# TrackieWay-OSS/TrackieLLM

Measured on AMD Instinct MI355X. Metric: cortex cycles/sec (frame+1s audio+128 tok), higher is better.
Workload: dtype int8 x q4_K/q6_K (i32 acc, f32 scales); 1 GPU; configs[3] fused cycle: YOLOv8n 640x640 frame (preprocess+network+NMS) + 1 s PCM (VAD + Whisper-tiny.en log-mel/encoder/16 forced decoder steps) + Mistral-7B Q4_K_M 64-token prefill and 128-token greedy decode, 3 concurrent HIP streams; concurrent_cycles_per_gpu=768, decode_groups=3, rows_per_llm_pass=256, layers=32, parallelism=replicas x1

## Files before the change

### include/tk/tk_audio.h

```cpp
#ifndef TK_MI355X_AUDIO_H
#define TK_MI355X_AUDIO_H

#include "tk_types.h"

#ifdef __cplusplus
extern "C" {
#endif

typedef struct tk_asr_whisper_context_s tk_asr_whisper_context_t;

typedef struct {
    tk_path_t* model_path;
    const char* language;
    bool translate_to_en;
    uint32_t sample_rate;
    void* user_data;
    int n_threads;
    int max_context;
    float word_threshold;
} tk_asr_whisper_config_t;

typedef struct {
    char* text;
    size_t text_length;
// ... 35 lines not shown
TK_API TK_NODISCARD tk_error_code_t tk_vad_silero_create(tk_vad_silero_context_t** out_context, const tk_vad_silero_config_t* config);
TK_API void tk_vad_silero_destroy(tk_vad_silero_context_t** context);
TK_API TK_NODISCARD tk_error_code_t tk_vad_silero_process_audio(tk_vad_silero_context_t* context, const int16_t* audio_data, size_t frame_count,
                                                                float* out_probability);
TK_API TK_NODISCARD tk_error_code_t tk_vad_silero_process_audio_with_events(tk_vad_silero_context_t* context, const int16_t* audio_data,
                                                                            size_t frame_count, tk_vad_silero_event_callback_t callback,
                                                                            void* user_data);
TK_API TK_NODISCARD tk_error_code_t tk_vad_silero_get_state(tk_vad_silero_context_t* context, tk_vad_silero_state_t* out_state);
TK_API TK_NODISCARD tk_error_code_t tk_vad_silero_reset(tk_vad_silero_context_t* context);
TK_API TK_NODISCARD tk_error_code_t tk_vad_silero_set_threshold(tk_vad_silero_context_t* context, float threshold);

typedef struct {
    int32_t n_mels, n_audio_ctx, n_audio_state, n_audio_head, n_audio_layer;
    int32_t n_text_ctx, n_text_state, n_text_head, n_text_layer, n_vocab;
} tk_mi355x_whisper_hparams_t;
TK_API TK_NODISCARD tk_error_code_t tk_mi355x_asr_create(tk_asr_whisper_context_t** out, const tk_mi355x_whisper_hparams_t* hp, uint64_t seed,
                                                         int device, int max_batch);
TK_API TK_NODISCARD tk_error_code_t tk_mi355x_asr_transcribe_tokens(tk_asr_whisper_context_t* ctx, int batch, const int16_t* pcm, int n_samples,
                                                                    int n_steps, int32_t* tokens_out, float* mel_out, float* enc_out,
                                                                    float* logits_out);
TK_API void tk_mi355x_asr_set_decode_steps(tk_asr_whisper_context_t* ctx, int n_steps);
TK_API TK_NODISCARD tk_error_code_t tk_mi355x_asr_set_reference_decode(tk_asr_whisper_context_t* ctx, int enable);
TK_API TK_NODISCARD tk_error_code_t tk_mi355x_asr_set_fast_contraction(tk_asr_whisper_context_t* ctx, int on);
TK_API TK_NODISCARD tk_error_code_t tk_mi355x_asr_transcribe_ref(tk_asr_whisper_context_t* ctx, const int16_t* pcm, int n_samples, int n_steps, float temperature,
                                                                 uint64_t seed, int32_t* tokens_out, float* logprobs_out, int32_t* result_len, int32_t* status);
TK_API int32_t tk_mi355x_asr_suppress_table(tk_asr_whisper_context_t* ctx, uint8_t* out, int32_t cap, int32_t* token_beg, int32_t* token_eot);
TK_API void tk_mi355x_asr_share_stats(const tk_asr_whisper_context_t* ctx, uint64_t* handles, uint64_t* batches, uint64_t* utterances, uint64_t* widest);
TK_API TK_NODISCARD tk_error_code_t tk_mi355x_asr_transcribe_policy(tk_asr_whisper_context_t* ctx, int batch, const int16_t* pcm, int n_samples,
                                                                    int n_steps, float temperature, uint64_t seed, int32_t* tokens_out,
                                                                    float* logprobs_out);
TK_API TK_NODISCARD tk_error_code_t tk_mi355x_asr_set_decode_policy(tk_asr_whisper_context_t* ctx, int enable, float temperature_inc,
                                                                    float entropy_thold, float logprob_thold, uint64_t seed);
TK_API void tk_mi355x_asr_last_decode(const tk_asr_whisper_context_t* ctx, float* temperature, float* avg_logprob, int32_t* attempts);
TK_API int tk_mi355x_asr_prompt_tokens(tk_asr_whisper_context_t* ctx, int32_t* out, int cap);
TK_API TK_NODISCARD tk_error_code_t tk_mi355x_asr_get_hparams(tk_asr_whisper_context_t* ctx, tk_mi355x_whisper_hparams_t* out);
TK_API TK_NODISCARD tk_error_code_t tk_mi355x_whisper_ggml_probe(const char* path, tk_mi355x_whisper_hparams_t* out, int32_t* n_tokens,
                                                                 int32_t* n_tensors);
TK_API TK_NODISCARD tk_error_code_t tk_mi355x_vad_onnx_probe(const char* path, int32_t* n_nodes, int32_t* n_initialisers, int32_t* n_state_inputs);
TK_API int tk_mi355x_vad_step(tk_vad_silero_context_t* ctx, float probability);
TK_API TK_NODISCARD tk_error_code_t tk_mi355x_vad_probabilities(tk_vad_silero_context_t* ctx, const float* windows, int n, float* out);

#ifdef __cplusplus
}
#endif
#endif
```

### trackiellm_amd/audio.py

```python
import ctypes as C

import numpy as np

from ._lib import check, lib
from .llm import _Path


class WhisperHP(C.Structure):
    _fields_ = [(n, C.c_int32) for n in ("n_mels", "n_audio_ctx", "n_audio_state", "n_audio_head", "n_audio_layer",
                                         "n_text_ctx", "n_text_state", "n_text_head", "n_text_layer", "n_vocab")]


def WHISPER_TINY_EN():
    return WhisperHP(80, 1500, 384, 6, 4, 448, 384, 6, 4, 51864)


class _AsrConfig(C.Structure):
    _fields_ = [("model_path", C.POINTER(_Path)), ("language", C.c_char_p), ("translate_to_en", C.c_bool), ("sample_rate", C.c_uint32),
                ("user_data", C.c_void_p), ("n_threads", C.c_int), ("max_context", C.c_int), ("word_threshold", C.c_float)]


class AsrResult(C.Structure):
    _fields_ = [("text", C.c_char_p), ("text_length", C.c_size_t), ("confidence", C.c_float), ("is_partial", C.c_bool)]

# ... 39 lines not shown
    def transcribe_policy(self, pcm, n_steps, temperature=0.0, seed=0):
        pcm = np.ascontiguousarray(pcm, np.int16)
        B, n = pcm.shape
        toks = np.zeros((B, n_steps), np.int32)
        lp = np.zeros((B, n_steps), np.float32)
        check(lib().tk_mi355x_asr_transcribe_policy(self.h, B, pcm.ctypes.data_as(C.c_void_p), n, n_steps, C.c_float(temperature), C.c_uint64(seed),
                                                    toks.ctypes.data_as(C.c_void_p), lp.ctypes.data_as(C.c_void_p)))
        return toks, lp

    def set_decode_policy(self, enable=True, temperature_inc=0.2, entropy_thold=2.4, logprob_thold=-1.0, seed=0):
        check(lib().tk_mi355x_asr_set_decode_policy(self.h, int(enable), C.c_float(temperature_inc), C.c_float(entropy_thold),
                                                    C.c_float(logprob_thold), C.c_uint64(seed)))

    def last_decode(self):
        t, a, n = C.c_float(0), C.c_float(0), C.c_int32(0)
        lib().tk_mi355x_asr_last_decode(self.h, C.byref(t), C.byref(a), C.byref(n))
        return t.value, a.value, n.value

    def set_reference_decode(self, enable=True):
        check(lib().tk_mi355x_asr_set_reference_decode(self.h, int(enable)))

    def set_fast_contraction(self, on=True):
        check(lib().tk_mi355x_asr_set_fast_contraction(self.h, 1 if on else 0))

    def transcribe_ref(self, pcm, n_steps, temperature=0.0, seed=0):
        pcm = np.ascontiguousarray(pcm, np.int16).reshape(-1)
        toks = np.zeros(n_steps, np.int32)
        lp = np.zeros(n_steps, np.float32)
        rl, st = C.c_int32(0), C.c_int32(0)
        check(lib().tk_mi355x_asr_transcribe_ref(self.h, pcm.ctypes.data_as(C.c_void_p), pcm.size, n_steps, C.c_float(temperature), C.c_uint64(seed),
                                                 toks.ctypes.data_as(C.c_void_p), lp.ctypes.data_as(C.c_void_p), C.byref(rl), C.byref(st)))
        return toks, lp, rl.value, st.value

    def suppress_table(self):
        beg, eot = C.c_int32(0), C.c_int32(0)
        n = lib().tk_mi355x_asr_suppress_table(self.h, None, 0, C.byref(beg), C.byref(eot))
        if n <= 0:
            return None, 0, 0
        tab = np.zeros(n, np.uint8)
        lib().tk_mi355x_asr_suppress_table(self.h, tab.ctypes.data_as(C.c_void_p), n, C.byref(beg), C.byref(eot))
        return tab, beg.value, eot.value

    def share_stats(self):
        v = [C.c_uint64(0) for _ in range(4)]
        lib().tk_mi355x_asr_share_stats(self.h, *[C.byref(x) for x in v])
        return tuple(int(x.value) for x in v)
# ... 184 lines not shown
```

### trackiellm_amd/csrc/abi/tk_abi_audio.cpp

```cpp
#include <math.h>
#include <stdio.h>
#include <stdlib.h>
#include <string.h>
#include <unistd.h>

#include <memory>
#include <string>
#include <vector>

#include "../audio/tk_audio_engine.h"
#include "../audio/tk_vad_graph.h"
#include "../audio/tk_whisper_ggml.h"
#include "tk/tk_audio.h"
#include "tk/tk_mi355x_ext.h"

#define TK_ASR_MAX_BUFFER (16000 * 30)

static tk_error_code_t afail(tk_error_code_t code, const std::string& why) {
    tk_error_set_detail("%s", why.c_str());
    return code;
}

static uint64_t seed_of(const std::string& p, uint64_t dflt) {
    size_t k = p.find("seed=");
// ... 4 lines not shown
static std::string file_identity(const std::string& path) {
    struct stat st;
    if (path.compare(0, 12, "synthetic://") == 0 || stat(path.c_str(), &st) != 0) return path;
    return path + "|" + std::to_string((long long)st.st_size) + "|" + std::to_string((long long)st.st_mtim.tv_sec) + "." + std::to_string((long long)st.st_mtim.tv_nsec) + "|" +
           std::to_string((unsigned long long)st.st_ino);
}

#include <chrono>
#include <condition_variable>
#include <deque>
#include <map>
#include <mutex>
#include <thread>

#define TK_ASR_SHARED_MAX_BATCH 32

struct AsrReq {
    const int16_t* pcm = nullptr;
    int n_samples = 0, n_steps = 0;
    std::vector<int32_t> prompt;
    bool policy = false;
    bool ref = false;
    bool fast = false;
    float temperature = 0.0f;
    uint64_t seed = 0;
    int32_t* tokens = nullptr;
    float* logprobs = nullptr;
    int32_t result_len = 0, status = 0;
    bool ok = false, done = false;
    std::string err;
};

struct SharedAsr {
    std::string key;
    TkWhisperModel model;
    std::vector<std::string> vocab;
    std::vector<uint8_t> suppress;
    int32_t token_beg = 0, token_eot = 0;
    std::unique_ptr<TkAsr> eng;
    bool scheduled = false;
    std::mutex mu;
    std::condition_variable cv_req, cv_done;
    std::deque<AsrReq*> q;
    std::thread th;
    bool stop = false;
    int handles = 0;
// ... 15 lines not shown
        if (eng && eng->max_batch >= want) return true;
        std::unique_ptr<TkAsr> ne(new TkAsr());
        if (!ne->init(&model, want)) { *err = ne->error; return false; }
        eng.swap(ne);
        return true;
    }
    void run() {
        std::unique_lock<std::mutex> lk(mu);
        for (;;) {
            cv_req.wait(lk, [&] { return stop || !q.empty(); });
            if (stop) break;
            if (handles > 1 && !q.front()->policy) {
                const auto until = std::chrono::steady_clock::now() + std::chrono::microseconds(1000);
                while ((int)q.size() < (handles < TK_ASR_SHARED_MAX_BATCH ? handles : TK_ASR_SHARED_MAX_BATCH) && !stop)
                    if (cv_req.wait_until(lk, until) == std::cv_status::timeout) break;
                if (stop) break;
            }
            std::vector<AsrReq*> job;
            AsrReq* first = q.front();
            if (first->policy) { job.push_back(first); q.pop_front(); }
            else
                for (auto it = q.begin(); it != q.end() && (int)job.size() < TK_ASR_SHARED_MAX_BATCH;) {
                    AsrReq* r = *it;
                    if (!r->policy && r->ref == first->ref && r->fast == first->fast && r->n_steps == first->n_steps && r->prompt == first->prompt) { job.push_back(r); it = q.erase(it); }
                    else ++it;
                }
            int cap = 1;
            while (cap < (int)job.size() || (cap < handles && cap < TK_ASR_SHARED_MAX_BATCH)) cap *= 2;
            lk.unlock();
            std::string err;
            std::unique_lock<std::mutex> el(eng_mu);
            bool ok = ensure_engine(cap, &err);
            if (ok) {
                eng->fast = first->fast;
                const int B = (int)job.size();
                int n_max = 0;
                for (AsrReq* r : job) n_max = r->n_samples > n_max ? r->n_samples : n_max;
                if (first->ref) {
                    std::vector<int16_t> pcm((size_t)B * (n_max > 0 ? n_max : 1), 0);
                    std::vector<int32_t> lens(B), toks((size_t)B * first->n_steps), rl(B), stt(B);
                    std::vector<float> lps((size_t)B * first->n_steps);
                    for (int b = 0; b < B; ++b) {
                        lens[b] = job[b]->n_samples;
                        if (job[b]->n_samples > 0) memcpy(&pcm[(size_t)b * n_max], job[b]->pcm, (size_t)job[b]->n_samples * sizeof(int16_t));
                    }
                    ok = eng->transcribe_ref(B, pcm.data(), n_max, lens.data(), first->prompt.data(), (int)first->prompt.size(), first->n_steps, first->temperature, first->seed,
                                             suppress.data(), token_beg, token_eot, toks.data(), lps.data(), rl.data(), stt.data());
                    for (int b = 0; ok && b < B; ++b) {
                        memcpy(job[b]->tokens, &toks[(size_t)b * first->n_steps], (size_t)first->n_steps * sizeof(int32_t));
                        if (job[b]->logprobs) memcpy(job[b]->logprobs, &lps[(size_t)b * first->n_steps], (size_t)first->n_steps * sizeof(float));
                        job[b]->result_len = rl[b];
                        job[b]->status = stt[b];
                    }
                } else if (first->policy) {
                    ok = eng->transcribe_policy(1, first->pcm, first->n_samples, first->prompt.data(), (int)first->prompt.size(), first->n_steps, first->temperature, first->seed,
                                                first->tokens, first->logprobs);
                } else if (B == 1) {
// ... 23 lines not shown
    }
    void submit(AsrReq* r) {
        std::unique_lock<std::mutex> lk(mu);
        q.push_back(r);
        cv_req.notify_all();
        cv_done.wait(lk, [&] { return r->done; });
    }
};

static std::mutex g_asr_mu;
static std::map<std::string, std::weak_ptr<SharedAsr>> g_asr_registry;

struct tk_asr_whisper_context_s {
    std::shared_ptr<SharedAsr> sh;
    std::vector<int16_t> buffer;
    size_t buffer_size = 0;
    bool has_partial = false;
    std::string last_text, language;
    int decode_steps = 16;
    int32_t sot = 0, nots = 0, eot = 0;
    bool multilingual = false, translate = false;
    bool forced_greedy = false;
    bool fast = false;
    bool policy_on = false;
    float temperature_inc = 0.2f, entropy_thold = 2.4f, logprob_thold = -1.0f;
    uint64_t policy_seed = 0;
    float last_temperature = 0.0f, last_avg_logprob = 0.0f;
    int last_attempts = 0;
    ~tk_asr_whisper_context_s() {
        if (sh) { std::lock_guard<std::mutex> lk(sh->mu); sh->handles--; }
    }
};

static const char* const k_whisper_langs[] = {
    "en", "zh", "de", "es", "ru", "ko", "fr", "ja", "pt", "tr", "pl", "ca", "nl", "ar", "sv", "it", "id", "hi", "fi", "vi", "he", "uk", "el", "ms", "cs",
    "ro", "da", "hu", "ta", "no", "th", "ur", "hr", "bg", "lt", "la", "mi", "ml", "cy", "sk", "te", "fa", "lv", "bn", "sr", "az", "sl", "kn", "et", "mk",
    "br", "eu", "is", "hy", "ne", "mn", "bs", "kk", "sq", "sw", "gl", "mr", "pa", "si", "km", "sn", "yo", "so", "af", "oc", "ka", "be", "tg", "sd", "gu",
    "am", "yi", "lo", "uz", "fo", "ht", "ps", "tk", "nn", "mt", "sa", "lb", "my", "bo", "tl", "mg", "as", "tt", "haw", "ln", "ha", "ba", "jw", "su", "yue"};

static int whisper_lang_id(const std::string& code) {
    for (int i = 0; i < (int)(sizeof k_whisper_langs / sizeof k_whisper_langs[0]); ++i)
        if (code == k_whisper_langs[i]) return i;
    return -1;
}

static bool asr_prompt(const tk_asr_whisper_context_s* c, std::vector<int32_t>* out, std::string* why, bool timestamps = false) {
// ... 102 lines not shown
    c->sot = 50257 + ml < v - 3 ? 50257 + ml : v - 3;
    c->nots = 50362 + ml < v - 1 ? 50362 + ml : v - 1;
    c->eot = 50256 + ml < v - 4 ? 50256 + ml : v - 4;
    c->multilingual = ml != 0;
    if (ml) {
        const int n_lang = v - 51865 + 99;
        c->eot = 50257; c->sot = 50258;
        c->nots = c->sot + 1 + n_lang + 5;
    }
    { std::lock_guard<std::mutex> hl(sh->mu); build_suppress(sh.get(), c.get()); }
    *out = c.release();
    return TK_SUCCESS;
}

static tk_error_code_t asr_run_ref(tk_asr_whisper_context_s* c, const int16_t* pcm, int n_samples, const std::vector<int32_t>& prompt, int n_steps, float temperature,
                                   uint64_t seed, int32_t* tokens_out, float* logprobs_out, int32_t* result_len, int32_t* status) {
    SharedAsr* sh = c->sh.get();
    const TkWhisperHP& h = sh->model.hp;
    if (sh->suppress.empty()) return afail(TK_ERROR_INFERENCE_FAILED, "this vocabulary has no timestamp tokens: the reference-parameter decode does not apply");
    if (n_samples < 0 || n_samples > h.n_samples()) return afail(TK_ERROR_INFERENCE_FAILED, "audio longer than the model window");
    if (prompt.empty() || (int)prompt.size() + n_steps > h.n_text_ctx) return afail(TK_ERROR_INFERENCE_FAILED, "prompt + steps exceed the text context");
    if (sh->scheduled) {
        AsrReq r;
        r.pcm = pcm; r.n_samples = n_samples; r.n_steps = n_steps; r.prompt = prompt; r.ref = true; r.fast = c->fast; r.policy = temperature > 0.0f; r.temperature = temperature; r.seed = seed;
        r.tokens = tokens_out; r.logprobs = logprobs_out;
        sh->submit(&r);
        if (!r.ok) return afail(TK_ERROR_INFERENCE_FAILED, r.err);
        if (result_len) *result_len = r.result_len;
        if (status) *status = r.status;
        return TK_SUCCESS;
    }
    std::lock_guard<std::mutex> lk(sh->eng_mu);
    const int32_t len = n_samples;
    int32_t rl = 0, stt = 0;
    sh->eng->fast = c->fast;
    if (!sh->eng->transcribe_ref(1, pcm, n_samples, &len, prompt.data(), (int)prompt.size(), n_steps, temperature, seed, sh->suppress.data(), sh->token_beg, sh->token_eot,
                                 tokens_out, logprobs_out, &rl, &stt))
        return afail(TK_ERROR_INFERENCE_FAILED, sh->eng->error);
    if (result_len) *result_len = rl;
    if (status) *status = stt;
    return TK_SUCCESS;
}

static tk_error_code_t asr_run(tk_asr_whisper_context_s* c, int batch, const int16_t* pcm, int n_samples, const std::vector<int32_t>& prompt, int n_steps, bool policy,
                               float temperature, uint64_t seed, int32_t* tokens_out, float* logprobs_out, std::vector<float>* mel, std::vector<float>* enc,
                               std::vector<float>* lg) {
    SharedAsr* sh = c->sh.get();
    if (sh->scheduled && batch == 1 && !mel && !enc && !lg) {
        AsrReq r;
        r.pcm = pcm; r.n_samples = n_samples; r.n_steps = n_steps; r.prompt = prompt; r.fast = c->fast; r.policy = policy; r.temperature = temperature; r.seed = seed;
        r.tokens = tokens_out; r.logprobs = logprobs_out;
        const TkWhisperHP& h = sh->model.hp;
        if (n_samples < 0 || n_samples > h.n_samples()) return afail(TK_ERROR_INFERENCE_FAILED, "audio longer than the model window");
        if (prompt.empty() || (int)prompt.size() + n_steps > h.n_text_ctx) return afail(TK_ERROR_INFERENCE_FAILED, "prompt + steps exceed the text context");
        sh->submit(&r);
        return r.ok ? TK_SUCCESS : afail(TK_ERROR_INFERENCE_FAILED, r.err);
    }
    std::lock_guard<std::mutex> lk(sh->eng_mu);
    std::string err;
    if (!sh->ensure_engine(batch, &err)) return afail(TK_ERROR_GPU_MEMORY, err);
    sh->eng->fast = c->fast;
    const bool ok = policy ? sh->eng->transcribe_policy(batch, pcm, n_samples, prompt.data(), (int)prompt.size(), n_steps, temperature, seed, tokens_out, logprobs_out)
                           : sh->eng->transcribe(batch, pcm, n_samples, prompt.data(), (int)prompt.size(), n_steps, tokens_out, mel, enc, lg);
    return ok ? TK_SUCCESS : afail(TK_ERROR_INFERENCE_FAILED, sh->eng->error);
}

extern "C" {

tk_error_code_t tk_asr_whisper_create(tk_asr_whisper_context_t** out_context, const tk_asr_whisper_config_t* config) {
    if (!out_context || !config || !config->model_path || !config->model_path->path_str) return TK_ERROR_INVALID_ARGUMENT;
    if (config->sample_rate != 16000) return afail(TK_ERROR_INVALID_ARGUMENT, "Whisper needs 16 kHz audio");
    const std::string path = config->model_path->path_str;
    tk_error_code_t rc = asr_new(out_context, tk_whisper_tiny_en(), path, seed_of(path, 6), tk_mi355x_get_default_device(), 1, true);
    if (rc == TK_SUCCESS && config->language) (*out_context)->language = config->language;
    if (rc == TK_SUCCESS) (*out_context)->translate = config->translate_to_en;
    const char* pol = getenv("TK_MI355X_ASR_POLICY");
    if (rc == TK_SUCCESS && pol && pol[0] == '1') (*out_context)->policy_on = true;
    return rc;
}

tk_error_code_t tk_mi355x_asr_create(tk_asr_whisper_context_t** out, const tk_mi355x_whisper_hparams_t* hp, uint64_t seed, int device, int max_batch) {
    if (!out || !hp) return TK_ERROR_INVALID_ARGUMENT;
    TkWhisperHP h{hp->n_mels, hp->n_audio_ctx, hp->n_audio_state, hp->n_audio_head, hp->n_audio_layer,
                  hp->n_text_ctx, hp->n_text_state, hp->n_text_head, hp->n_text_layer, hp->n_vocab};
// ... 23 lines not shown
        bool ok = false;
        for (const auto& t : g.tensors)
            if (t.name == man.t[i].name) { ok = t.count == man.t[i].rows * man.t[i].cols; break; }
        if (!ok) return afail(TK_ERROR_MODEL_VERIFICATION_FAILED, "tensor " + man.t[i].name + " is missing or has the wrong size");
    }
    return TK_SUCCESS;
}

void tk_asr_whisper_destroy(tk_asr_whisper_context_t** context) {
    if (!context || !*context) return;
    delete *context;
    *context = nullptr;
}

void tk_mi355x_asr_share_stats(const tk_asr_whisper_context_t* c, uint64_t* handles, uint64_t* batches, uint64_t* utterances, uint64_t* widest) {
    if (!c || !c->sh) return;
    std::lock_guard<std::mutex> lk(c->sh->mu);
    if (handles) *handles = (uint64_t)c->sh->handles;
    if (batches) *batches = c->sh->n_batches;
    if (utterances) *utterances = c->sh->n_utts;
    if (widest) *widest = c->sh->widest;
}

tk_error_code_t tk_mi355x_asr_set_fast_contraction(tk_asr_whisper_context_t* c, int on) {
    if (!c) return TK_ERROR_INVALID_ARGUMENT;
    c->fast = on != 0;
    return TK_SUCCESS;
}

tk_error_code_t tk_mi355x_asr_set_reference_decode(tk_asr_whisper_context_t* c, int enable) {
    if (!c) return TK_ERROR_INVALID_ARGUMENT;
    c->forced_greedy = enable == 0;
    return TK_SUCCESS;
}

tk_error_code_t tk_mi355x_asr_transcribe_ref(tk_asr_whisper_context_t* c, const int16_t* pcm, int n_samples, int n_steps, float temperature, uint64_t seed, int32_t* tokens_out,
                                             float* logprobs_out, int32_t* result_len, int32_t* status) {
    if (!c || (!pcm && n_samples > 0) || !tokens_out || n_steps <= 0) return TK_ERROR_INVALID_ARGUMENT;
    std::vector<int32_t> prompt;
    std::string why;
    if (!asr_prompt(c, &prompt, &why, true)) return afail(TK_ERROR_INFERENCE_FAILED, why);
    return asr_run_ref(c, pcm, n_samples, prompt, n_steps, temperature, seed, tokens_out, logprobs_out, result_len, status);
}

int32_t tk_mi355x_asr_suppress_table(tk_asr_whisper_context_t* c, uint8_t* out, int32_t cap, int32_t* token_beg, int32_t* token_eot) {
    if (!c) return -1;
// ... 2 lines not shown
    if (out) for (int32_t i = 0; i < n && i < cap; ++i) out[i] = c->sh->suppress[(size_t)i];
    if (token_beg) *token_beg = c->sh->token_beg;
    if (token_eot) *token_eot = c->sh->token_eot;
    return n;
}

void tk_mi355x_asr_set_decode_steps(tk_asr_whisper_context_t* ctx, int n_steps) {
    if (ctx && n_steps > 0) ctx->decode_steps = n_steps;
}

tk_error_code_t tk_mi355x_asr_transcribe_tokens(tk_asr_whisper_context_t* c, int batch, const int16_t* pcm, int n_samples, int n_steps,
                                                int32_t* tokens_out, float* mel_out, float* enc_out, float* logits_out) {
    if (!c || (!pcm && n_samples > 0) || !tokens_out || n_steps <= 0) return TK_ERROR_INVALID_ARGUMENT;
    std::vector<int32_t> prompt;
    std::string why;
    if (!asr_prompt(c, &prompt, &why)) return afail(TK_ERROR_INFERENCE_FAILED, why);
    std::vector<float> mel, enc, lg;
    tk_error_code_t rc = asr_run(c, batch, pcm, n_samples, prompt, n_steps, false, 0.0f, 0, tokens_out, nullptr, mel_out ? &mel : nullptr, enc_out ? &enc : nullptr,
                                 logits_out ? &lg : nullptr);
    if (rc != TK_SUCCESS) return rc;
    if (mel_out) memcpy(mel_out, mel.data(), mel.size() * 4);
    if (enc_out) memcpy(enc_out, enc.data(), enc.size() * 4);
    if (logits_out) memcpy(logits_out, lg.data(), lg.size() * 4);
    return TK_SUCCESS;
}

tk_error_code_t tk_mi355x_asr_transcribe_policy(tk_asr_whisper_context_t* c, int batch, const int16_t* pcm, int n_samples, int n_steps, float temperature,
                                                uint64_t seed, int32_t* tokens_out, float* logprobs_out) {
    if (!c || (!pcm && n_samples > 0) || !tokens_out || n_steps <= 0) return TK_ERROR_INVALID_ARGUMENT;
    std::vector<int32_t> prompt;
    std::string why;
    if (!asr_prompt(c, &prompt, &why)) return afail(TK_ERROR_INFERENCE_FAILED, why);
    return asr_run(c, batch, pcm, n_samples, prompt, n_steps, true, temperature, seed, tokens_out, logprobs_out, nullptr, nullptr, nullptr);
}

tk_error_code_t tk_mi355x_asr_set_decode_policy(tk_asr_whisper_context_t* c, int enable, float temperature_inc, float entropy_thold, float logprob_thold, uint64_t seed) {
    if (!c) return TK_ERROR_INVALID_ARGUMENT;
    c->policy_on = enable != 0;
    c->temperature_inc = temperature_inc; c->entropy_thold = entropy_thold; c->logprob_thold = logprob_thold; c->policy_seed = seed;
    return TK_SUCCESS;
}

void tk_mi355x_asr_last_decode(const tk_asr_whisper_context_t* c, float* temperature, float* avg_logprob, int32_t* attempts) {
    if (!c) return;
    if (temperature) *temperature = c->last_temperature;
    if (avg_logprob) *avg_logprob = c->last_avg_logprob;
// ... 314 lines not shown
```

### trackiellm_amd/csrc/audio/tk_audio_engine.h

```cpp
#ifndef TK_AUDIO_ENGINE_H
#define TK_AUDIO_ENGINE_H

#include <hip/hip_runtime.h>
#include <stdint.h>

#include <string>
#include <vector>

#include "../common/tk_whisper_graph.h"

size_t tk_attend1_lds_bytes(int Tk, int d, int nh);
bool tk_attend1_ok(const float* k, const float* v, int B, int Tk, int64_t q_bstride, int64_t kv_bstride, int d, int nh);
bool tk_launch_attend1(const float* q, const float* k, const float* v, float* out, int B, int Tk, int64_t q_bstride, int64_t kv_bstride, int d, int nh, float* img,
                       hipStream_t s);

class TkWhisperModel {
public:
    TkWhisperHP hp{};
    TkWhManifest man;
    int device = 0;
    std::vector<float*> w;
    std::vector<uint8_t*> wt;
    bool prepare_tiles();
    int tensor_of(const float* dev_ptr) const;
    std::string error;
    ~TkWhisperModel();
    bool init(const TkWhisperHP& hp, int device);
    bool fill_synthetic(uint64_t seed);
    bool set_tensor(int idx, const float* host, size_t n);
    bool load_file(const char* path);
    bool load_ggml(class TkWhisperGgml& g);
};

class TkAsr {
public:
    TkWhisperModel* model = nullptr;
    int max_batch = 1;
    bool fast = false;
    std::string error;
    hipStream_t stream = nullptr;
    ~TkAsr();
    bool init(TkWhisperModel* m, int max_batch);
    bool transcribe(int B, const int16_t* pcm, int n_samples, const int32_t* prompt, int n_prompt, int n_steps, int32_t* tokens_out,
                    std::vector<float>* mel_out, std::vector<float>* enc_out, std::vector<float>* first_logits);
    bool transcribe_policy(int B, const int16_t* pcm, int n_samples, const int32_t* prompt, int n_prompt, int n_steps, float temperature, uint64_t seed,
                           int32_t* tokens_out, float* logprobs_out);
    bool transcribe_ref(int B, const int16_t* pcm, int n_samples, const int32_t* n_samples_row, const int32_t* prompt, int n_prompt, int n_steps, float temperature,
                        uint64_t seed, const uint8_t* suppress, int32_t token_beg, int32_t token_eot, int32_t* tokens_out, float* logprobs_out, int32_t* result_len,
                        int32_t* status);

private:
    friend struct TkAudioGpuOps;
    float* arena = nullptr;
    size_t arena_floats = 0, arena_used = 0;
    std::string launch_error;
    int16_t* pcm_dev = nullptr;
    size_t pcm_cap = 0;
    struct { bool on = false; float temp = 0.0f; uint64_t seed = 0; float* logprob = nullptr; int step = 0;
             bool filtered = false; int first_step = 0; const uint8_t* suppress = nullptr; int32_t* state = nullptr; int32_t beg = 0, eot = 0, tid0 = 0; } pick;
    uint8_t* suppress_dev = nullptr;
    std::vector<uint8_t> suppress_host;
// ... 22 lines not shown
```

### trackiellm_amd/csrc/audio/tk_audio_engine.hip

```cpp
#include "tk_audio_engine.h"
#include "tk_whisper_ggml.h"

#include <stdio.h>
#include <string.h>

#include "../nn/tk_gemm_tiled.h"
#include "../nn/tk_nn_kernels.h"

static inline hipError_t tk_create_perception_stream(hipStream_t* s) {
    int lo = 0, hi = 0;
    if (hipDeviceGetStreamPriorityRange(&lo, &hi) != hipSuccess) return hipStreamCreateWithFlags(s, hipStreamNonBlocking);
    return hipStreamCreateWithPriority(s, hipStreamNonBlocking, hi);
}

#define HIPQ(expr)                                                                              \
    do {                                                                                        \
        hipError_t e__ = (expr);                                                                \
        if (e__ != hipSuccess) {                                                                \
            char b__[256];                                                                      \
            snprintf(b__, sizeof b__, "%s failed: %s (%s:%d)", #expr, hipGetErrorString(e__), __FILE__, __LINE__); \
            error = b__;                                                                        \
            return false;                                                                       \
        }                                                                                       \
    } while (0)
// ... 18 lines not shown
    const int f = (int)(i % nb);
    const float re = ri[r * 2 * nb + f], im = ri[r * 2 * nb + nb + f];
    out[i] = tk_fmaf(re, re, im * im);
}

__global__ __launch_bounds__(1024) void k_logmel_finish(float* mel, int per_b) {
    __shared__ float red[16];
    float* m = mel + (int64_t)blockIdx.x * per_b;
    float mx = -INFINITY;
    for (int i = threadIdx.x; i < per_b; i += 1024) {
        const float v = tk_log10f(tk_fmaxf(m[i], 1e-10f));
        m[i] = v;
        mx = tk_fmaxf(mx, v);
    }
    for (int s = 32; s >= 1; s >>= 1) mx = tk_fmaxf(mx, __shfl_xor(mx, s, 64));
    if ((threadIdx.x & 63) == 0) red[threadIdx.x >> 6] = mx;
    __syncthreads();
    mx = red[0];
    for (int w = 1; w < 16; ++w) mx = tk_fmaxf(mx, red[w]);
    const float floor_v = mx - 8.0f;
    for (int i = threadIdx.x; i < per_b; i += 1024) m[i] = (tk_fmaxf(m[i], floor_v) + 4.0f) * 0.25f;
}


#define TK_AT1_CK 64
#define TK_AT1_NS 3
__device__ __forceinline__ void at1_wait_vmcnt(int n) {
#define TK_VMW(k) case k: __builtin_amdgcn_s_waitcnt(0x0F70 | ((k) & 15) | (((k) >> 4) << 14)); break;
    switch (n) {
        TK_VMW(0) TK_VMW(1) TK_VMW(2) TK_VMW(3) TK_VMW(4) TK_VMW(5) TK_VMW(6) TK_VMW(7) TK_VMW(8) TK_VMW(9) TK_VMW(10) TK_VMW(11) TK_VMW(12)
        TK_VMW(13) TK_VMW(14) TK_VMW(15) TK_VMW(16)
        default: __builtin_amdgcn_s_waitcnt(0x0F70); break;
    }
#undef TK_VMW
}
__global__ __launch_bounds__(256) void k_attend1(const float* q, const float* k, const float* v, float* out, int Tk, int64_t q_bstride, int64_t kv_bstride, int d,
                                                 int hd, float scale, float* img ) {
    extern __shared__ __attribute__((aligned(16))) float att1_lds[];
    __shared__ float red[4];
    float* vring = att1_lds;
    float* sc = att1_lds + (size_t)TK_AT1_NS * TK_AT1_CK * hd;
    float* qs = sc + Tk;
    const int h = blockIdx.x, b = blockIdx.y, t0 = threadIdx.x, lane = t0 & 63;
    const int wave = __builtin_amdgcn_readfirstlane(t0 >> 6);
    const float* qp = q + (int64_t)b * q_bstride + (int64_t)h * hd;
    const float* kp = k + (int64_t)b * kv_bstride + (int64_t)h * hd;
// ... 494 lines not shown
}

bool TkAsr::transcribe(int B, const int16_t* pcm, int n_samples, const int32_t* prompt, int n_prompt, int n_steps, int32_t* tokens_out,
                       std::vector<float>* mel_out, std::vector<float>* enc_out, std::vector<float>* first_logits) {
    const TkWhisperHP& h = model->hp;
    if (B < 1 || B > max_batch) { error = "batch larger than the ASR context was created for"; return false; }
    if (n_samples < 0 || n_samples > h.n_samples()) { error = "audio longer than the model window"; return false; }
    if (n_prompt < 1 || n_prompt + n_steps > h.n_text_ctx) { error = "prompt + steps exceed the text context"; return false; }
    HIPQ(hipSetDevice(model->device));
    size_t need = (size_t)B * (n_samples > 0 ? n_samples : 1);
    if (need > pcm_cap) need = (size_t)max_batch * (size_t)h.n_samples();
    if (need > pcm_cap) {
        if (pcm_dev) (void)hipFree(pcm_dev);
        pcm_dev = nullptr;
        HIPQ(hipMalloc((void**)&pcm_dev, need * 2));
        pcm_cap = need;
    }
    if (n_samples > 0) HIPQ(hipMemcpyAsync(pcm_dev, pcm, (size_t)B * n_samples * 2, hipMemcpyHostToDevice, stream));
    arena_used = 0;
    launch_error.clear();
    TkAudioGpuOps ops{this, stream};
    TkWhisperGraph<TkAudioGpuOps> g{h, model->man, model->w.data()};
    ops.long_ok = true;
    float* ml = g.mel(ops, pcm_dev, B, n_samples, n_samples);
    float* enc = g.encode(ops, ml, B);
    auto st = g.begin_decode(ops, enc, B);
    ops.long_ok = false;
    HIPQ(hipGetLastError());
    if (mel_out) { mel_out->resize((size_t)B * h.n_frames() * h.n_mels); HIPQ(hipMemcpyAsync(mel_out->data(), ml, mel_out->size() * 4, hipMemcpyDeviceToHost, stream)); }
    if (enc_out) { enc_out->resize((size_t)B * h.n_audio_ctx * h.n_audio_state); HIPQ(hipMemcpyAsync(enc_out->data(), enc, enc_out->size() * 4, hipMemcpyDeviceToHost, stream)); }
    const int total = n_prompt + n_steps - 1;
    const size_t tab_ints = ((size_t)n_prompt + 2 * (size_t)total) * B;
    ops.drop_image();
    if (arena_used + tab_ints + 64 > arena_floats) { error = "ASR arena too small for the decode tables"; return false; }
    int32_t* tab = ops.alloc_i32(tab_ints);
    int32_t* tok_tab = tab;
    int32_t* pos_tab = tab + (size_t)n_prompt * B;
    int32_t* out_tab = pos_tab + (size_t)total * B;
    std::vector<int32_t> host_tab(((size_t)n_prompt + total) * B);
    for (int p = 0; p < n_prompt; ++p)
        for (int b = 0; b < B; ++b) host_tab[(size_t)p * B + b] = prompt[p];
    for (int p = 0; p < total; ++p)
        for (int b = 0; b < B; ++b) host_tab[((size_t)n_prompt + p) * B + b] = p;
    HIPQ(hipMemcpyAsync(tok_tab, host_tab.data(), host_tab.size() * 4, hipMemcpyHostToDevice, stream));
    int steps_run = n_steps;
    std::vector<int32_t> st_host;
    for (int p = 0; p < total; ++p) {
        st.tok = p < n_prompt ? tok_tab + (size_t)p * B : out_tab + (size_t)(p - 1) * B;
        st.pos = pos_tab + (size_t)p * B;
        st.next = out_tab + (size_t)p * B;
        g.decode_step(ops, st, p);
        if (p == n_prompt - 1 && first_logits) {
// ... 91 lines not shown
```

### trackiellm_amd/csrc/common/tk_whisper_graph.h

```cpp
#ifndef TK_WHISPER_GRAPH_H
#define TK_WHISPER_GRAPH_H

#include <math.h>
#include <stdint.h>

#include <string>
#include <vector>

#include "tk_exact_math.h"
#include "tk_gemm_desc.h"
#include "tk_ggml_blocks.h"

#define TK_WH_NFFT 400
#define TK_WH_HOP 160
#define TK_WH_NBINS 201
#define TK_WH_LN_EPS 1e-5f

struct TkWhisperHP {
    int32_t n_mels, n_audio_ctx, n_audio_state, n_audio_head, n_audio_layer;
    int32_t n_text_ctx, n_text_state, n_text_head, n_text_layer, n_vocab;
    int n_frames() const { return 2 * n_audio_ctx; }
    int n_samples() const { return n_frames() * TK_WH_HOP; }
};

// ... 111 lines not shown
static inline void tk_vad_synth(uint64_t seed, int window, int hidden, float* w1, float* b1, float* w2, float* b2) {
    const float s1 = tk_sqrtf(tk_divf(1.0f, (float)window)) * 8.0f, s2 = tk_sqrtf(tk_divf(1.0f, (float)hidden)) * 4.0f;
    for (int64_t i = 0; i < (int64_t)window * hidden; ++i) w1[i] = s1 * tk_synth_normal(seed, 7001, (uint64_t)i);
    for (int i = 0; i < hidden; ++i) b1[i] = 0.1f * tk_synth_normal(seed, 7002, (uint64_t)i);
    for (int i = 0; i < hidden; ++i) w2[i] = s2 * tk_synth_normal(seed, 7003, (uint64_t)i);
    b2[0] = -1.0f;
}

template <class Ops>
struct TkWhisperGraph {
    const TkWhisperHP& h;
    const TkWhManifest& m;
    float* const* W;

    static TkGemm lin(const float* A, int M, int K, int lda, const float* Wt, const float* bias, int N, float* C, int ldc, int act = 0,
                      const float* res = nullptr, int ldr = 0) {
        TkGemm g{};
        g.A = A; g.B = Wt; g.C = C; g.bias = bias; g.residual = res;
        g.M = M; g.N = N; g.K = K; g.lda = lda; g.ldb = K; g.ldc = ldc; g.ldr = ldr;
        g.b_kn = 0; g.act = act; g.alpha = 1.0f; g.batch = 1;
        return g;
    }

    float* mel(Ops& o, const int16_t* pcm, int B, int n_samples, int pcm_stride) const {
        const int T = h.n_frames();
        float* fr = o.alloc((size_t)B * T * TK_WH_NFFT);
        o.frames(pcm, B, n_samples, pcm_stride, h.n_samples(), T, W[m.hann], fr);
        float* ri = o.alloc((size_t)B * T * 2 * TK_WH_NBINS);
        o.gemm(lin(fr, B * T, TK_WH_NFFT, TK_WH_NFFT, W[m.dft], nullptr, 2 * TK_WH_NBINS, ri, 2 * TK_WH_NBINS));
        float* pw = o.alloc((size_t)B * T * TK_WH_NBINS);
        o.power(ri, B * T, TK_WH_NBINS, pw);
        float* ml = o.alloc((size_t)B * T * h.n_mels);
        o.gemm(lin(pw, B * T, TK_WH_NBINS, TK_WH_NBINS, W[m.melw], nullptr, h.n_mels, ml, h.n_mels));
        o.logmel_finish(ml, B, T * h.n_mels);
        return ml;
    }

    static int score_pitch(int Tk) { return (Tk + 31) & ~31; }
    void attention(Ops& o, const float* q, const float* k, const float* v, float* out, int B, int Tq, int Tk, int64_t q_bstride, int64_t kv_bstride,
                   int d, int nh, float* scores) const {
        const int hd = d / nh;
        if (Tq == 1 && o.attend1(q, k, v, out, B, Tk, q_bstride, kv_bstride, d, nh)) return;
        if (Tq > 1 && o.attend_fused(q, k, v, out, B, Tq, Tk, q_bstride, kv_bstride, d, nh)) return;
        const int Tp = score_pitch(Tk);
        TkGemm s{};
        s.A = q; s.B = k; s.C = scores; s.M = Tq; s.N = Tk; s.K = hd; s.lda = d; s.ldb = d; s.ldc = Tp; s.b_kn = 0; s.act = 0;
        s.alpha = tk_divf(1.0f, tk_sqrtf((float)hd));
        s.batch = B * nh; s.batch_inner = nh;
        s.sA = hd; s.sB = hd; s.sC = (int64_t)Tq * Tp;
        s.sA2 = q_bstride; s.sB2 = kv_bstride; s.sC2 = (int64_t)nh * Tq * Tp;
        o.gemm(s);
        o.softmax_rows(scores, B * nh * Tq, Tk, Tp);
        TkGemm p{};
        p.A = scores; p.B = v; p.C = out; p.M = Tq; p.N = hd; p.K = Tk; p.lda = Tp; p.ldb = d; p.ldc = d; p.b_kn = 1; p.act = 0; p.alpha = 1.0f;
        p.batch = B * nh; p.batch_inner = nh;
        p.sA = (int64_t)Tq * Tp; p.sB = hd; p.sC = hd;
        p.sA2 = (int64_t)nh * Tq * Tp; p.sB2 = kv_bstride; p.sC2 = q_bstride;
        o.gemm(p);
    }

    float* encode(Ops& o, const float* ml, int B) const {
        const int T = h.n_frames(), Tc = h.n_audio_ctx, d = h.n_audio_state, nh = h.n_audio_head;
        float* col1 = o.alloc((size_t)B * T * 3 * h.n_mels);
        o.im2col1d(ml, B, T, h.n_mels, h.n_mels, 3, 1, 1, col1);
        float* x1 = o.alloc((size_t)B * T * d);
        o.gemm(lin(col1, B * T, 3 * h.n_mels, 3 * h.n_mels, W[m.conv1_w], W[m.conv1_b], d, x1, d, TK_ACT_GELU));
        float* col2 = o.alloc((size_t)B * Tc * 3 * d);
        o.im2col1d(x1, B, T, d, d, 3, 2, 1, col2);
        float* x = o.alloc((size_t)B * Tc * d);
        o.gemm(lin(col2, B * Tc, 3 * d, 3 * d, W[m.conv2_w], W[m.conv2_b], d, x, d, TK_ACT_GELU));
        o.add_rows(x, W[m.enc_pos], B * Tc, d, Tc);
        float* hb = o.alloc((size_t)B * Tc * d);
        float* q = o.alloc((size_t)B * Tc * d);
        float* k = o.alloc((size_t)B * Tc * d);
        float* v = o.alloc((size_t)B * Tc * d);
        float* at = o.alloc((size_t)B * Tc * d);
        float* ff = o.alloc((size_t)B * Tc * 4 * d);
        float* sc = o.alloc((size_t)B * nh * Tc * score_pitch(Tc));
        const int R = B * Tc;
        for (int l = 0; l < h.n_audio_layer; ++l) {
            const TkWhLayerIdx& L = m.enc[l];
            o.layernorm(x, R, d, W[L.ln1_w], W[L.ln1_b], hb);
            o.gemm(lin(hb, R, d, d, W[L.q_w], W[L.q_b], d, q, d));
            o.gemm(lin(hb, R, d, d, W[L.k_w], nullptr, d, k, d));
            o.gemm(lin(hb, R, d, d, W[L.v_w], W[L.v_b], d, v, d));
            attention(o, q, k, v, at, B, Tc, Tc, (int64_t)Tc * d, (int64_t)Tc * d, d, nh, sc);
            o.gemm(lin(at, R, d, d, W[L.o_w], W[L.o_b], d, x, d, 0, x, d));
            o.layernorm(x, R, d, W[L.ln2_w], W[L.ln2_b], hb);
            { TkGemm g1 = lin(hb, R, d, d, W[L.fc1_w], W[L.fc1_b], 4 * d, ff, 4 * d, TK_ACT_GELU); g1.c_feeds_linear = 1; o.gemm(g1); }
            o.gemm(lin(ff, R, 4 * d, 4 * d, W[L.fc2_w], W[L.fc2_b], d, x, d, 0, x, d));
        }
        float* y = o.alloc((size_t)R * d);
        o.layernorm(x, R, d, W[m.enc_ln_w], W[m.enc_ln_b], y);
        return y;
// ... 61 lines not shown
```

Measured before the change: 187.7 cycles/s.

## Compute Whisper mel and conv front-end only over audible frames

Whisper pads audio to a 30 s window, but for 1 s of PCM most mel frames are identical padding. The engine now computes the log-mel and the two conv layers only over the audible frames plus a small margin. It then expands the conv output to the full 1500-row context by replicating a representative padding row, fusing this with the positional-embedding add. This removes most of the front-end mel and conv GEMM work. The encoder blocks still run over the full context, and correctness rests on the padded rows being constant, which a new conv_probe hook and full_window toggle let tests check.

```diff
diff --git a/include/tk/tk_audio.h b/include/tk/tk_audio.h
--- a/include/tk/tk_audio.h
+++ b/include/tk/tk_audio.h
@@ -81,6 +81,8 @@
 TK_API void tk_mi355x_asr_set_decode_steps(tk_asr_whisper_context_t* ctx, int n_steps);
 TK_API TK_NODISCARD tk_error_code_t tk_mi355x_asr_set_reference_decode(tk_asr_whisper_context_t* ctx, int enable);
 TK_API TK_NODISCARD tk_error_code_t tk_mi355x_asr_set_fast_contraction(tk_asr_whisper_context_t* ctx, int on);
+TK_API TK_NODISCARD tk_error_code_t tk_mi355x_asr_set_full_window(tk_asr_whisper_context_t* ctx, int on);
+TK_API TK_NODISCARD tk_error_code_t tk_mi355x_asr_conv_probe(tk_asr_whisper_context_t* ctx, int batch, const int16_t* pcm, int n_samples, float* x_out);
 TK_API TK_NODISCARD tk_error_code_t tk_mi355x_asr_transcribe_ref(tk_asr_whisper_context_t* ctx, const int16_t* pcm, int n_samples, int n_steps, float temperature,
                                                                  uint64_t seed, int32_t* tokens_out, float* logprobs_out, int32_t* result_len, int32_t* status);
 TK_API int32_t tk_mi355x_asr_suppress_table(tk_asr_whisper_context_t* ctx, uint8_t* out, int32_t cap, int32_t* token_beg, int32_t* token_eot);
diff --git a/trackiellm_amd/audio.py b/trackiellm_amd/audio.py
--- a/trackiellm_amd/audio.py
+++ b/trackiellm_amd/audio.py
@@ -85,6 +85,16 @@
 
     def set_fast_contraction(self, on=True):
         check(lib().tk_mi355x_asr_set_fast_contraction(self.h, 1 if on else 0))
+
+    def set_full_window(self, on=True):
+        check(lib().tk_mi355x_asr_set_full_window(self.h, 1 if on else 0))
+
+    def conv_output(self, pcm):
+        pcm = np.ascontiguousarray(pcm, np.int16)
+        B, n = pcm.shape
+        x = np.empty((B, self.hp.n_audio_ctx, self.hp.n_audio_state), np.float32)
+        check(lib().tk_mi355x_asr_conv_probe(self.h, B, pcm.ctypes.data_as(C.c_void_p), n, x.ctypes.data_as(C.c_void_p)))
+        return x
 
     def transcribe_ref(self, pcm, n_steps, temperature=0.0, seed=0):
         pcm = np.ascontiguousarray(pcm, np.int16).reshape(-1)
diff --git a/trackiellm_amd/csrc/abi/tk_abi_audio.cpp b/trackiellm_amd/csrc/abi/tk_abi_audio.cpp
--- a/trackiellm_amd/csrc/abi/tk_abi_audio.cpp
+++ b/trackiellm_amd/csrc/abi/tk_abi_audio.cpp
@@ -50,6 +50,7 @@
     bool policy = false;
     bool ref = false;
     bool fast = false;
+    bool full_window = false;
     float temperature = 0.0f;
     uint64_t seed = 0;
     int32_t* tokens = nullptr;
@@ -111,7 +112,7 @@
             else
                 for (auto it = q.begin(); it != q.end() && (int)job.size() < TK_ASR_SHARED_MAX_BATCH;) {
                     AsrReq* r = *it;
-                    if (!r->policy && r->ref == first->ref && r->fast == first->fast && r->n_steps == first->n_steps && r->prompt == first->prompt) { job.push_back(r); it = q.erase(it); }
+                    if (!r->policy && r->ref == first->ref && r->fast == first->fast && r->full_window == first->full_window && r->n_steps == first->n_steps && r->prompt == first->prompt) { job.push_back(r); it = q.erase(it); }
                     else ++it;
                 }
             int cap = 1;
@@ -122,6 +123,7 @@
             bool ok = ensure_engine(cap, &err);
             if (ok) {
                 eng->fast = first->fast;
+                eng->full_window = first->full_window;
                 const int B = (int)job.size();
                 int n_max = 0;
                 for (AsrReq* r : job) n_max = r->n_samples > n_max ? r->n_samples : n_max;
@@ -191,6 +193,7 @@
     bool multilingual = false, translate = false;
     bool forced_greedy = false;
     bool fast = false;
+    bool full_window = false;
     bool policy_on = false;
     float temperature_inc = 0.2f, entropy_thold = 2.4f, logprob_thold = -1.0f;
     uint64_t policy_seed = 0;
@@ -339,7 +342,7 @@
     if (prompt.empty() || (int)prompt.size() + n_steps > h.n_text_ctx) return afail(TK_ERROR_INFERENCE_FAILED, "prompt + steps exceed the text context");
     if (sh->scheduled) {
         AsrReq r;
-        r.pcm = pcm; r.n_samples = n_samples; r.n_steps = n_steps; r.prompt = prompt; r.ref = true; r.fast = c->fast; r.policy = temperature > 0.0f; r.temperature = temperature; r.seed = seed;
+        r.pcm = pcm; r.n_samples = n_samples; r.n_steps = n_steps; r.prompt = prompt; r.ref = true; r.fast = c->fast; r.full_window = c->full_window; r.policy = temperature > 0.0f; r.temperature = temperature; r.seed = seed;
         r.tokens = tokens_out; r.logprobs = logprobs_out;
         sh->submit(&r);
         if (!r.ok) return afail(TK_ERROR_INFERENCE_FAILED, r.err);
@@ -351,6 +354,7 @@
     const int32_t len = n_samples;
     int32_t rl = 0, stt = 0;
     sh->eng->fast = c->fast;
+    sh->eng->full_window = c->full_window;
     if (!sh->eng->transcribe_ref(1, pcm, n_samples, &len, prompt.data(), (int)prompt.size(), n_steps, temperature, seed, sh->suppress.data(), sh->token_beg, sh->token_eot,
                                  tokens_out, logprobs_out, &rl, &stt))
         return afail(TK_ERROR_INFERENCE_FAILED, sh->eng->error);
@@ -365,7 +369,7 @@
     SharedAsr* sh = c->sh.get();
     if (sh->scheduled && batch == 1 && !mel && !enc && !lg) {
         AsrReq r;
-        r.pcm = pcm; r.n_samples = n_samples; r.n_steps = n_steps; r.prompt = prompt; r.fast = c->fast; r.policy = policy; r.temperature = temperature; r.seed = seed;
+        r.pcm = pcm; r.n_samples = n_samples; r.n_steps = n_steps; r.prompt = prompt; r.fast = c->fast; r.full_window = c->full_window; r.policy = policy; r.temperature = temperature; r.seed = seed;
         r.tokens = tokens_out; r.logprobs = logprobs_out;
         const TkWhisperHP& h = sh->model.hp;
         if (n_samples < 0 || n_samples > h.n_samples()) return afail(TK_ERROR_INFERENCE_FAILED, "audio longer than the model window");
@@ -377,6 +381,7 @@
     std::string err;
     if (!sh->ensure_engine(batch, &err)) return afail(TK_ERROR_GPU_MEMORY, err);
     sh->eng->fast = c->fast;
+    sh->eng->full_window = c->full_window;
     const bool ok = policy ? sh->eng->transcribe_policy(batch, pcm, n_samples, prompt.data(), (int)prompt.size(), n_steps, temperature, seed, tokens_out, logprobs_out)
                            : sh->eng->transcribe(batch, pcm, n_samples, prompt.data(), (int)prompt.size(), n_steps, tokens_out, mel, enc, lg);
     return ok ? TK_SUCCESS : afail(TK_ERROR_INFERENCE_FAILED, sh->eng->error);
@@ -446,6 +451,12 @@
     if (widest) *widest = c->sh->widest;
 }
 
+tk_error_code_t tk_mi355x_asr_set_full_window(tk_asr_whisper_context_t* c, int on) {
+    if (!c) return TK_ERROR_INVALID_ARGUMENT;
+    c->full_window = on != 0;
+    return TK_SUCCESS;
+}
+
 tk_error_code_t tk_mi355x_asr_set_fast_contraction(tk_asr_whisper_context_t* c, int on) {
     if (!c) return TK_ERROR_INVALID_ARGUMENT;
     c->fast = on != 0;
@@ -494,6 +505,27 @@
     if (mel_out) memcpy(mel_out, mel.data(), mel.size() * 4);
     if (enc_out) memcpy(enc_out, enc.data(), enc.size() * 4);
     if (logits_out) memcpy(logits_out, lg.data(), lg.size() * 4);
+    return TK_SUCCESS;
+}
+
+tk_error_code_t tk_mi355x_asr_conv_probe(tk_asr_whisper_context_t* c, int batch, const int16_t* pcm, int n_samples, float* x_out) {
+    if (!c || (!pcm && n_samples > 0) || !x_out || batch < 1) return TK_ERROR_INVALID_ARGUMENT;
+    std::vector<int32_t> prompt;
+    std::string why;
+    if (!asr_prompt(c, &prompt, &why)) return afail(TK_ERROR_INFERENCE_FAILED, why);
+    SharedAsr* sh = c->sh.get();
+    std::lock_guard<std::mutex> lk(sh->eng_mu);
+    std::string err;
+    if (!sh->ensure_engine(batch, &err)) return afail(TK_ERROR_GPU_MEMORY, err);
+    sh->eng->fast = c->fast;
+    sh->eng->full_window = c->full_window;
+    std::vector<float> x;
+    std::vector<int32_t> toks((size_t)batch);
+    sh->eng->conv_out = &x;
+    const bool ok = sh->eng->transcribe(batch, pcm, n_samples, prompt.data(), (int)prompt.size(), 1, toks.data(), nullptr, nullptr, nullptr);
+    sh->eng->conv_out = nullptr;
+    if (!ok) return afail(TK_ERROR_INFERENCE_FAILED, sh->eng->error);
+    memcpy(x_out, x.data(), x.size() * 4);
     return TK_SUCCESS;
 }
 
diff --git a/trackiellm_amd/csrc/audio/tk_audio_engine.h b/trackiellm_amd/csrc/audio/tk_audio_engine.h
--- a/trackiellm_amd/csrc/audio/tk_audio_engine.h
+++ b/trackiellm_amd/csrc/audio/tk_audio_engine.h
@@ -37,6 +37,8 @@
     TkWhisperModel* model = nullptr;
     int max_batch = 1;
     bool fast = false;
+    bool full_window = false;
+    std::vector<float>* conv_out = nullptr;
     std::string error;
     hipStream_t stream = nullptr;
     ~TkAsr();
diff --git a/trackiellm_amd/csrc/audio/tk_audio_engine.hip b/trackiellm_amd/csrc/audio/tk_audio_engine.hip
--- a/trackiellm_amd/csrc/audio/tk_audio_engine.hip
+++ b/trackiellm_amd/csrc/audio/tk_audio_engine.hip
@@ -64,6 +64,15 @@
     for (int i = threadIdx.x; i < per_b; i += 1024) m[i] = (tk_fmaxf(m[i], floor_v) + 4.0f) * 0.25f;
 }
 
+
+__global__ void k_expand_add_rows(const float* xc, int Tn2, int ur, const float* pos, int Tc, int D, int64_t total, float* x) {
+    for (int64_t i = (int64_t)blockIdx.x * blockDim.x + threadIdx.x; i < total; i += (int64_t)gridDim.x * blockDim.x) {
+        const int64_t r = i / D;
+        const int c = (int)(i % D), b = (int)(r / Tc), u = (int)(r % Tc);
+        const int src = u < ur ? u : (u == Tc - 1 ? Tn2 - 1 : ur);
+        x[i] = xc[((int64_t)b * Tn2 + src) * D + c] + pos[(int64_t)u * D + c];
+    }
+}
 
 #define TK_AT1_CK 64
 #define TK_AT1_NS 3
@@ -604,12 +613,40 @@
     TkAudioGpuOps ops{this, stream};
     TkWhisperGraph<TkAudioGpuOps> g{h, model->man, model->w.data()};
     ops.long_ok = true;
-    float* ml = g.mel(ops, pcm_dev, B, n_samples, n_samples);
-    float* enc = g.encode(ops, ml, B);
+    const int T = h.n_frames(), Tc = h.n_audio_ctx, d = h.n_audio_state;
+    const int Tn = full_window ? T : g.audible_frames(n_samples);
+    float* ml = g.mel(ops, pcm_dev, B, n_samples, n_samples, Tn);
+    float* x;
+    if (Tn == T) {
+        x = g.conv_front(ops, ml, B, T);
+        ops.add_rows(x, model->w[(size_t)model->man.enc_pos], B * Tc, d, Tc);
+    } else {
+        const float* xc = g.conv_front(ops, ml, B, Tn);
+        x = ops.alloc((size_t)B * Tc * d);
+        const int64_t total = (int64_t)B * Tc * d;
+        hipLaunchKernelGGL(k_expand_add_rows, dim3((unsigned)((total + 255) / 256)), dim3(256), 0, stream, xc, Tn / 2, g.representative_row(Tn), model->w[(size_t)model->man.enc_pos],
+                           Tc, d, total, x);
+    }
+    if (conv_out) {
+        conv_out->resize((size_t)B * Tc * d);
+        HIPQ(hipMemcpyAsync(conv_out->data(), x, conv_out->size() * 4, hipMemcpyDeviceToHost, stream));
+        HIPQ(hipStreamSynchronize(stream));
+    }
+    float* enc = g.encode_blocks(ops, x, B);
     auto st = g.begin_decode(ops, enc, B);
     ops.long_ok = false;
     HIPQ(hipGetLastError());
-    if (mel_out) { mel_out->resize((size_t)B * h.n_frames() * h.n_mels); HIPQ(hipMemcpyAsync(mel_out->data(), ml, mel_out->size() * 4, hipMemcpyDeviceToHost, stream)); }
+    if (mel_out && Tn == T) { mel_out->resize((size_t)B * T * h.n_mels); HIPQ(hipMemcpyAsync(mel_out->data(), ml, mel_out->size() * 4, hipMemcpyDeviceToHost, stream)); }
+    if (mel_out && Tn < T) {
+        std::vector<float> part((size_t)B * Tn * h.n_mels);
+        HIPQ(hipMemcpyAsync(part.data(), ml, part.size() * 4, hipMemcpyDeviceToHost, stream));
+        HIPQ(hipStreamSynchronize(stream));
+        mel_out->resize((size_t)B * T * h.n_mels);
+        const size_t row = (size_t)h.n_mels;
+        for (int b = 0; b < B; ++b)
+            for (int t = 0; t < T; ++t)
+                memcpy(mel_out->data() + ((size_t)b * T + t) * row, part.data() + ((size_t)b * Tn + (t < Tn ? t : Tn - 1)) * row, row * sizeof(float));
+    }
     if (enc_out) { enc_out->resize((size_t)B * h.n_audio_ctx * h.n_audio_state); HIPQ(hipMemcpyAsync(enc_out->data(), enc, enc_out->size() * 4, hipMemcpyDeviceToHost, stream)); }
     const int total = n_prompt + n_steps - 1;
     const size_t tab_ints = ((size_t)n_prompt + 2 * (size_t)total) * B;
diff --git a/trackiellm_amd/csrc/common/tk_whisper_graph.h b/trackiellm_amd/csrc/common/tk_whisper_graph.h
--- a/trackiellm_amd/csrc/common/tk_whisper_graph.h
+++ b/trackiellm_amd/csrc/common/tk_whisper_graph.h
@@ -157,8 +157,17 @@
         return g;
     }
 
-    float* mel(Ops& o, const int16_t* pcm, int B, int n_samples, int pcm_stride) const {
+    int audible_frames(int n_samples) const {
         const int T = h.n_frames();
+        int tz = (n_samples + TK_WH_NFFT / 2 + TK_WH_HOP - 1) / TK_WH_HOP;
+        if (tz < 2) tz = 2;
+        const int Tn = 2 * ((tz + 3) / 2) + 4;
+        return Tn < T ? Tn : T;
+    }
+    static int representative_row(int Tn) { return (Tn - 4) / 2; }
+
+    float* mel(Ops& o, const int16_t* pcm, int B, int n_samples, int pcm_stride, int T = 0) const {
+        if (T <= 0) T = h.n_frames();
         float* fr = o.alloc((size_t)B * T * TK_WH_NFFT);
         o.frames(pcm, B, n_samples, pcm_stride, h.n_samples(), T, W[m.hann], fr);
         float* ri = o.alloc((size_t)B * T * 2 * TK_WH_NBINS);
@@ -194,8 +203,8 @@
         o.gemm(p);
     }
 
-    float* encode(Ops& o, const float* ml, int B) const {
-        const int T = h.n_frames(), Tc = h.n_audio_ctx, d = h.n_audio_state, nh = h.n_audio_head;
+    float* conv_front(Ops& o, const float* ml, int B, int T) const {
+        const int Tc = T / 2, d = h.n_audio_state;
         float* col1 = o.alloc((size_t)B * T * 3 * h.n_mels);
         o.im2col1d(ml, B, T, h.n_mels, h.n_mels, 3, 1, 1, col1);
         float* x1 = o.alloc((size_t)B * T * d);
@@ -204,7 +213,17 @@
         o.im2col1d(x1, B, T, d, d, 3, 2, 1, col2);
         float* x = o.alloc((size_t)B * Tc * d);
         o.gemm(lin(col2, B * Tc, 3 * d, 3 * d, W[m.conv2_w], W[m.conv2_b], d, x, d, TK_ACT_GELU));
-        o.add_rows(x, W[m.enc_pos], B * Tc, d, Tc);
+        return x;
+    }
+
+    float* encode(Ops& o, const float* ml, int B) const {
+        float* x = conv_front(o, ml, B, h.n_frames());
+        o.add_rows(x, W[m.enc_pos], B * h.n_audio_ctx, h.n_audio_state, h.n_audio_ctx);
+        return encode_blocks(o, x, B);
+    }
+
+    float* encode_blocks(Ops& o, float* x, int B) const {
+        const int Tc = h.n_audio_ctx, d = h.n_audio_state, nh = h.n_audio_head;
         float* hb = o.alloc((size_t)B * Tc * d);
         float* q = o.alloc((size_t)B * Tc * d);
         float* k = o.alloc((size_t)B * Tc * d);
```

After: 189.0 cycles/s, median of 6. About the same (+0.7%).
